# arkiven4/glow-tts

Hardware: AMD Instinct MI355X
Metric: mel_frames_per_sec_train_step (higher is better)
Workload: dtype bf16; 1 GPU; configs/base.json, LJSpeech-shaped synthetic batches, B=32/GPU, T_x<=150, T_y<=800, bf16 GEMMs; batch_per_gpu=32, T_x=150, T_y=800, batches_rotated=8, padded_frames_per_gpu_step=25600, rows_layout=ragged, graphs_captured=6, parallelism=dp1 (utterance-sharded, RCCL gradient all-reduce, fp32 on the wire), launch=one HIP graph per step (one per ragged-row bucket, captured up front)

## Files before the change

glow-tts_amd/csrc/wn_stack.hip:

```cpp
#include "common.h"
#include "internal.h"
#include "mfma_frag.h"
#include "../../include/glowtts_hip.h"

namespace {

constexpr int H = 192, TAPS = 5, NLMAX = 4;
constexpr int BM = 64;
constexpr int AP = H + 8;
constexpr int XR = BM + TAPS - 1;
constexpr int RING = 3, RING1 = RING;
constexpr int RB = 2 * RING - 1, RB1 = RB;
#ifndef WNS_PHASES
#define WNS_PHASES 0
#endif
#if WNS_PHASES
__device__ unsigned long long g_wns_ph[2 * 1024 * 48];
#define PH(i) do { if ((threadIdx.x == 0 || threadIdx.x == 256) && blockIdx.x < 1024)                                                \
                     g_wns_ph[((threadIdx.x >> 8) * 1024 + blockIdx.x) * 48 + (i)] = __builtin_amdgcn_s_memtime(); } while (0)
#else
#define PH(i) do { } while (0)
#endif
constexpr int KK2 = H / 16;
constexpr int STACK_LDS = (2 * XR + BM) * AP * 2;
constexpr int FWD_BIAS_FLOATS = NLMAX * 2 * H + (NLMAX - 1) * H;
constexpr int FWD_AFF_FLOATS = 2 * NLMAX * H;
constexpr int STACK_FWD_LDS = STACK_LDS + 2 * BM * AP * 2 + FWD_BIAS_FLOATS * 4;
constexpr int STACK_FWD_LDS_AFF = STACK_FWD_LDS + FWD_AFF_FLOATS * 4;
constexpr int CPR = H / 8;

template <typename T>
__device__ __forceinline__ const T* pinned(const T* p) { asm volatile("" : "+s"(p)); return p; }
__device__ __forceinline__ int wave_scalar()
{
  int w = __builtin_amdgcn_readfirstlane((int)(threadIdx.x >> 6));
  asm volatile("" : "+s"(w));
  return w;
}

template <typename T>
__device__ __forceinline__ T pick(T const (&arr)[NLMAX], int i)
{
  return i == 0 ? arr[0] : (i == 1 ? arr[1] : (i == 2 ? arr[2] : arr[3]));
}

template <int COND, bool DROP, int NBM, bool SAVE = true>
__global__ __launch_bounds__(256) void gt_wn_stack_fwd_kernel(gt_wn_stack_fwd_args a, uint32_t drop_thresh, float drop_scale)
{
  constexpr int BMv = 32 * NBM, XRv = BMv + TAPS - 1;
  constexpr int RINGv = NBM == 1 ? RING1 : RING;
  extern __shared__ __attribute__((aligned(16))) unsigned char smem[];
  const unsigned long long t_begin = stamp_begin(a);
  PH(0);
  const uint32_t seed_x = a.seed_dev ? *a.seed_dev : 0u;
  const int lane = threadIdx.x & 63, wave = threadIdx.x >> 6;
  const int r = lane & 31, h = lane >> 5;
  const int n_layers = a.n_layers, R = a.R;
  const int halo = 2 * (n_layers - 1);
  const int own = BMv - 2 * halo;
  const int s0 = blockIdx.x * own - halo;
  bf16_t* Xc = reinterpret_cast<bf16_t*>(smem);
  bf16_t* Xn = Xc + XR * AP;
  bf16_t* At = Xn + XR * AP;
  bf16_t* Tl = At + BM * AP;
  bf16_t* Sl = Tl + BM * AP;
  float* Bs = reinterpret_cast<float*>(Sl + BM * AP);
  constexpr int KS = H / 16, NBT = 2 * H / 32, NIT = 3 * TAPS;

  uint4 ring[RINGv][4][3];
  float rm2;
  auto w_frag = [&](const bf16_t* W, int it, int ks, int bn) {
    const int kg = it / TAPS, tap = it - kg * TAPS;
    return ldfrag_global(W, (tap * NBT + 3 * wave + bn) * KS + kg * 4 + ks, lane);
  };
  auto w_load_l = [&](const bf16_t* W, int it, uint4 (&dst)[4][3]) {
#pragma unroll
    for (int ks = 0; ks < 4; ++ks)
#pragma unroll
      for (int bn = 0; bn < 3; ++bn) dst[ks][bn] = w_frag(W, it, ks, bn);
  };
  {
    const bf16_t* x0 = static_cast<const bf16_t*>(a.x0);
    constexpr int NX = (XR * CPR + 255) / 256, NB = (FWD_BIAS_FLOATS / 4 + 255) / 256;
    uint4 xin[NX];
    float4 bin[NB];
    float4 ain[(FWD_AFF_FLOATS / 4 + 255) / 256];
    if (COND == 2) {
      const int O = H * n_layers;
#pragma unroll
      for (int i = 0; i < (FWD_AFF_FLOATS / 4 + 255) / 256; ++i) {
        const int idx = threadIdx.x + 256 * i;
        ain[i] = make_float4(0.f, 0.f, 0.f, 0.f);
        if (idx < O / 4) ain[i] = reinterpret_cast<const float4*>(a.aff_w)[idx];
        else if (idx < 2 * O / 4) ain[i] = reinterpret_cast<const float4*>(a.aff_b)[idx - O / 4];
      }
    }
#pragma unroll
    for (int i = 0; i < NX; ++i) {
      const int chunk = threadIdx.x + 256 * i, u = chunk / CPR, c8 = chunk - u * CPR, gm = s0 - 2 + u;
      xin[i] = make_uint4(0, 0, 0, 0);
      if (u < XRv && gm >= 0 && gm < R) xin[i] = *reinterpret_cast<const uint4*>(x0 + (size_t)gm * H + c8 * 8);
    }
#pragma unroll
    for (int i = 0; i < NB; ++i) {
      const int idx = threadIdx.x + 256 * i;
      bin[i] = make_float4(0.f, 0.f, 0.f, 0.f);
      if (idx < NLMAX * 2 * H / 4) {
        const int l = idx / (2 * H / 4), o = idx - l * (2 * H / 4);
        if (l < n_layers) bin[i] = reinterpret_cast<const float4*>(pick(a.b_in, l))[o];
      } else if (idx < FWD_BIAS_FLOATS / 4) {
        const int q = idx - NLMAX * 2 * H / 4, l = q / (H / 4), o = q - l * (H / 4);
        if (l < n_layers - 1) bin[i] = reinterpret_cast<const float4*>(pick(a.b_res, l))[o];
      }
    }
    {
      const int m = s0 + 32 * (wave >> 1) + r;
      rm2 = (m >= 0 && m < R) ? a.rowmask[m] : 0.0f;
    }
    {
      const bf16_t* W10 = static_cast<const bf16_t*>(a.w_in[0]);
#pragma unroll
      for (int p = 0; p < RINGv - 1; ++p) w_load_l(W10, p, ring[p]);
    }
#pragma unroll
    for (int i = 0; i < NX; ++i) {
      const int chunk = threadIdx.x + 256 * i, u = chunk / CPR, c8 = chunk - u * CPR;
      if (u < XRv) *reinterpret_cast<uint4*>(Xc + u * AP + c8 * 8) = xin[i];
    }
#pragma unroll
    for (int i = 0; i < NB; ++i) {
      const int idx = threadIdx.x + 256 * i;
      if (idx < FWD_BIAS_FLOATS / 4) reinterpret_cast<float4*>(Bs)[idx] = bin[i];
    }
    if (COND == 2) {
#pragma unroll
      for (int i = 0; i < (FWD_AFF_FLOATS / 4 + 255) / 256; ++i) {
        const int idx = threadIdx.x + 256 * i;
        if (idx < 2 * H * n_layers / 4) reinterpret_cast<float4*>(Bs + FWD_BIAS_FLOATS)[idx] = ain[i];
      }
    }
    if (threadIdx.x < 4 * 24) {
      const int q = threadIdx.x / 24, c8 = threadIdx.x - q * 24, u = q < 2 ? q : XRv - 4 + q;
      *reinterpret_cast<uint4*>(Xn + u * AP + c8 * 8) = make_uint4(0, 0, 0, 0);
    }
  }
  __syncthreads();
  PH(1);

  int cb[NBM] = {};
  float sg[NBM][2] = {};
  if (COND == 1) {
#pragma unroll
    for (int bm = 0; bm < NBM; ++bm) {
      const int m = s0 + 32 * bm + r, mc = m < 0 ? 0 : (m >= R ? R - 1 : m);
      cb[bm] = a.B > 0 ? gt_row_batch(a.row0, a.B, mc, a.Tp) : mc;
    }
  }
  if (COND == 2) {
#pragma unroll
    for (int bm = 0; bm < NBM; ++bm) {
      const int m = s0 + 32 * bm + r;
      if (m >= 0 && m < R) { const float2 v = *reinterpret_cast<const float2*>(a.aff_sig + 2 * (size_t)m); sg[bm][0] = v.x; sg[bm][1] = v.y; }
    }
  }

  for (int layer = 0; layer < n_layers; ++layer) {
    const bool last = layer == n_layers - 1;
    const bf16_t* W1 = static_cast<const bf16_t*>(pick(a.w_in, layer));
    const bf16_t* W2 = static_cast<const bf16_t*>(pick(a.w_res, layer));
    const float* bias1 = Bs + layer * 2 * H;
    const float* bias2 = Bs + NLMAX * 2 * H + layer * H;
    bf16_t* Tt = static_cast<bf16_t*>(pick(a.gate_t, layer));
    bf16_t* Ss = static_cast<bf16_t*>(pick(a.gate_s, layer));
    bf16_t* xo = static_cast<bf16_t*>(pick(a.x_out, layer));
    const uint32_t seed = (a.drop_seed + (uint32_t)layer) ^ seed_x;

    f32x16_t acc[3][NBM];
    acc_zero(acc);

    auto w_load = [&](int it, uint4 (&dst)[4][3]) { w_load_l(W1, it, dst); };
#pragma unroll
    for (int it = 0; it < NIT; ++it) {
      const int kg = it / TAPS, tap = it - kg * TAPS;
      w_load(it + RINGv - 1 < NIT ? it + RINGv - 1 : NIT - 1, ring[(it + RINGv - 1) % RINGv]);
      __builtin_amdgcn_sched_barrier(0);
      const bf16_t* xsb = Xc + (r + tap) * AP + 8 * h + kg * 64;
#pragma unroll
      for (int ks = 0; ks < 4; ++ks) {
        bf16x8_t bx[NBM];
#pragma unroll
        for (int bm = 0; bm < NBM; ++bm) bx[bm] = *reinterpret_cast<const bf16x8_t*>(xsb + 32 * bm * AP + ks * 16);
#pragma unroll
        for (int bn = 0; bn < 3; ++bn)
#pragma unroll
          for (int bm = 0; bm < NBM; ++bm)
            acc[bn][bm] = __builtin_amdgcn_mfma_f32_32x32x16_bf16(asfrag(ring[it % RINGv][ks][bn]), bx[bm], acc[bn][bm], 0, 0, 0);
      }
      __builtin_amdgcn_sched_barrier(0);
    }

    PH(2 + 6 * layer);
    int tid_e = threadIdx.x;
    asm volatile("" : "+v"(tid_e));
    const int r_e = tid_e & 31, h_e = (tid_e >> 5) & 1, wave_e = tid_e >> 6;
    const int wn2 = wave & 1, wm2 = wave >> 1;
    const bool st2 = wm2 < NBM;
    constexpr int R2 = KK2 / 2;
    uint4 ring2[R2][3];
    if (!last && st2) {
#pragma unroll
      for (int kk = 0; kk < R2; ++kk)
#pragma unroll
        for (int bn = 0; bn < 3; ++bn) ring2[kk][bn] = ldfrag_global(W2, (3 * wn2 + bn) * KK2 + kk, lane);
    }

    bf16_t* acts = static_cast<bf16_t*>(a.acts) + layer * H;
    const float* cond = COND == 1 ? a.cond + (size_t)layer * 2 * H : nullptr;
    const int aff_O = H * n_layers, aff_par = (2 * H * layer) / aff_O, aff_off = (2 * H * layer) - aff_par * aff_O;
    const float* Aw = Bs + FWD_BIAS_FLOATS + aff_off;
    const float* Ab = Aw + aff_O;
#pragma unroll
    for (int bn = 0; bn < 3; ++bn)
#pragma unroll
      for (int g = 0; g < 2; ++g) {
        const int c = 16 * (3 * wave_e + bn) + 8 * g + 4 * h_e;
        const float4 bt = *reinterpret_cast<const float4*>(bias1 + c), bs = *reinterpret_cast<const float4*>(bias1 + H + c);
        const float btv[4] = {bt.x, bt.y, bt.z, bt.w}, bsv[4] = {bs.x, bs.y, bs.z, bs.w};
#pragma unroll
        for (int bm = 0; bm < NBM; ++bm) {
          const int t = 32 * bm + r_e, m = s0 + t;
          float ctv[4] = {}, csv[4] = {};
          if (COND == 1) {
            const float* cp = cond + (size_t)cb[bm] * a.ldc + c;
            const float4 ct = *reinterpret_cast<const float4*>(cp), cs = *reinterpret_cast<const float4*>(cp + H);
            ctv[0] = ct.x; ctv[1] = ct.y; ctv[2] = ct.z; ctv[3] = ct.w; csv[0] = cs.x; csv[1] = cs.y; csv[2] = cs.z; csv[3] = cs.w;
          }
          if (COND == 2) {
            const float pv = aff_par ? sg[bm][1] : sg[bm][0];
            const float4 wt = *reinterpret_cast<const float4*>(Aw + c), ws = *reinterpret_cast<const float4*>(Aw + H + c);
            const float4 bt2 = *reinterpret_cast<const float4*>(Ab + c), bs2 = *reinterpret_cast<const float4*>(Ab + H + c);
            ctv[0] = bt2.x + pv * wt.x; ctv[1] = bt2.y + pv * wt.y; ctv[2] = bt2.z + pv * wt.z; ctv[3] = bt2.w + pv * wt.w;
            csv[0] = bs2.x + pv * ws.x; csv[1] = bs2.y + pv * ws.y; csv[2] = bs2.z + pv * ws.z; csv[3] = bs2.w + pv * ws.w;
          }
          float tt[4], ss[4], aa[4];
#pragma unroll
          for (int j = 0; j < 4; ++j) {
            float vt = acc[bn][bm][4 * g + j] + btv[j], vs = acc[bn][bm][4 * g + j + 8] + bsv[j];
            if (DROP) {
              bool kt, ks;
              drop_keep_gate(seed, m, c + j, drop_thresh16(drop_thresh), kt, ks);
              vt = kt ? vt * drop_scale : 0.0f;
              vs = ks ? vs * drop_scale : 0.0f;
            }
            vt += ctv[j]; vs += csv[j];
            tt[j] = tanhf_(vt); ss[j] = sigmoidf_(vs); aa[j] = tt[j] * ss[j];
          }
          if (SAVE) {
            *reinterpret_cast<uint2*>(Tl + t * AP + c) = pack4(tt[0], tt[1], tt[2], tt[3]);
            *reinterpret_cast<uint2*>(Sl + t * AP + c) = pack4(ss[0], ss[1], ss[2], ss[3]);
          }
          *reinterpret_cast<uint2*>(At + t * AP + c) = pack4(aa[0], aa[1], aa[2], aa[3]);
        }
      }
    PH(3 + 6 * layer);
    __syncthreads();
    PH(4 + 6 * layer);
    auto store_gate_tiles = [&]() {
      constexpr int NC = (BM * CPR + 255) / 256, NP = 2;
#pragma unroll 1
      for (int i0 = 0; i0 < NC; i0 += NP) {
        uint4 vt[NP], vs[NP], va[NP];
#pragma unroll
        for (int i = 0; i < NP; ++i) {
          const int idx = tid_e + 256 * (i0 + i), row = idx / CPR, c8 = idx - row * CPR, t = halo + row;
          vt[i] = vs[i] = va[i] = make_uint4(0, 0, 0, 0);
          if (idx < own * CPR) {
            if (SAVE) { vt[i] = *reinterpret_cast<const uint4*>(Tl + t * AP + c8 * 8); vs[i] = *reinterpret_cast<const uint4*>(Sl + t * AP + c8 * 8); }
            va[i] = *reinterpret_cast<const uint4*>(At + t * AP + c8 * 8);
          }
        }
#pragma unroll
        for (int i = 0; i < NP; ++i) {
          const int idx = tid_e + 256 * (i0 + i), row = idx / CPR, c8 = idx - row * CPR, m = s0 + halo + row;
          if (idx < own * CPR && m < R) {
            if (SAVE) {
              *reinterpret_cast<uint4*>(Tt + (size_t)m * H + c8 * 8) = vt[i];
              *reinterpret_cast<uint4*>(Ss + (size_t)m * H + c8 * 8) = vs[i];
            }
            *reinterpret_cast<uint4*>(acts + (size_t)m * a.ldacts + c8 * 8) = va[i];
          }
        }
      }
    };
    if (last) store_gate_tiles();
    if (last) break;

    f32x16_t acc2[3];
    acc_zero(acc2);
    if (st2) {
      const bf16_t* ab = At + (32 * wm2 + r) * AP + 8 * h;
#pragma unroll
      for (int kk = 0; kk < KK2; ++kk) {
        const bf16x8_t bfm = *reinterpret_cast<const bf16x8_t*>(ab + kk * 16);
#pragma unroll
        for (int bn = 0; bn < 3; ++bn) {
          acc2[bn] = __builtin_amdgcn_mfma_f32_32x32x16_bf16(asfrag(ring2[kk % R2][bn]), bfm, acc2[bn], 0, 0, 0);
          if (R2 < KK2 && kk + R2 < KK2) ring2[kk % R2][bn] = ldfrag_global(W2, (3 * wn2 + bn) * KK2 + kk + R2, lane);
        }
      }
    }
    PH(5 + 6 * layer);
    {
      const bf16_t* W1n = static_cast<const bf16_t*>(pick(a.w_in, layer + 1));
#pragma unroll
      for (int p = 0; p < RINGv - 1; ++p) w_load_l(W1n, p, ring[p]);
    }
    store_gate_tiles();
    if (st2) {
      const int t = 32 * wm2 + r;
      const float rm = rm2;
#pragma unroll
      for (int bn = 0; bn < 3; ++bn)
#pragma unroll
        for (int g = 0; g < 4; ++g) {
          const int n = 32 * (3 * wn2 + bn) + 8 * g + 4 * h;
          const float4 b2 = *reinterpret_cast<const float4*>(bias2 + n);
          float xv[4];
          unpack4(*reinterpret_cast<const uint2*>(Xc + (t + 2) * AP + n), xv);
          const uint2 v = pack4((acc2[bn][4 * g] + b2.x + xv[0]) * rm, (acc2[bn][4 * g + 1] + b2.y + xv[1]) * rm,
                                (acc2[bn][4 * g + 2] + b2.z + xv[2]) * rm, (acc2[bn][4 * g + 3] + b2.w + xv[3]) * rm);
          *reinterpret_cast<uint2*>(Xn + (t + 2) * AP + n) = v;
        }
    }
    __syncthreads();
    PH(6 + 6 * layer);
    bf16_t* tmp = Xc; Xc = Xn; Xn = tmp;
    if (SAVE) {
      constexpr int NC = (BM * CPR + 255) / 256, NP = 3;
#pragma unroll 1
      for (int i0 = 0; i0 < NC; i0 += NP) {
        uint4 vx[NP];
#pragma unroll
        for (int i = 0; i < NP; ++i) {
          const int idx = tid_e + 256 * (i0 + i), row = idx / CPR, c8 = idx - row * CPR;
          vx[i] = make_uint4(0, 0, 0, 0);
          if (idx < own * CPR) vx[i] = *reinterpret_cast<const uint4*>(Xc + (halo + row + 2) * AP + c8 * 8);
        }
#pragma unroll
        for (int i = 0; i < NP; ++i) {
          const int idx = tid_e + 256 * (i0 + i), row = idx / CPR, c8 = idx - row * CPR, m = s0 + halo + row;
          if (idx < own * CPR && m < R) *reinterpret_cast<uint4*>(xo + (size_t)m * H + c8 * 8) = vx[i];
        }
      }
    }
    if (threadIdx.x < 4 * 24) {
      const int q = threadIdx.x / 24, c8 = threadIdx.x - q * 24, u = q < 2 ? q : XRv - 4 + q;
      *reinterpret_cast<uint4*>(Xn + u * AP + c8 * 8) = make_uint4(0, 0, 0, 0);
    }
    PH(7 + 6 * layer);
  }
  PH(40);
  stamp_end(a, t_begin);
}

constexpr int BWD_THREADS = 512;
constexpr int DP = 2 * H + 8;
constexpr int EX_BYTES = 4 * 3 * 16 * 64 * 4;
constexpr int BWD_DT = XR * DP * 2;
static_assert(EX_BYTES <= BWD_DT, "the exchange buffer lives in the d pre tile");
constexpr int SBWD_LDS = BWD_DT + 4 * BM * AP * 2;

template <bool DROP>
__device__ __forceinline__ void gate_bwd4(const float (&dd)[4], const float (&t)[4], const float (&s)[4], uint32_t seed, int m, int n,
                                          uint32_t thresh, float scale, uint2& pt, uint2& ps, uint2& ct, uint2& cs)
{
  float gt[4], gs[4];
#pragma unroll
  for (int j = 0; j < 4; ++j) { gt[j] = dd[j] * s[j] * (1.0f - t[j] * t[j]); gs[j] = dd[j] * t[j] * s[j] * (1.0f - s[j]); }
  ct = pack4(gt[0], gt[1], gt[2], gt[3]); cs = pack4(gs[0], gs[1], gs[2], gs[3]);
  if (DROP) {
#pragma unroll
    for (int j = 0; j < 4; ++j) {
      bool kt, ks;
      drop_keep_gate(seed, m, n + j, drop_thresh16(thresh), kt, ks);
      gt[j] = kt ? gt[j] * scale : 0.0f;
      gs[j] = ks ? gs[j] * scale : 0.0f;
    }
  }
  pt = pack4(gt[0], gt[1], gt[2], gt[3]); ps = pack4(gs[0], gs[1], gs[2], gs[3]);
}

constexpr int B_NS = 2 * H / 64, B_NIT = B_NS * TAPS, B_KS = 2 * H / 16, B_NBT = H / 32;

template <int NB> constexpr int bwd_b0() { return NB == 2 ? 0 : 2; }

template <int NB>
__device__ __forceinline__ void bwd_w_load(const bf16_t* W1, int it, int wn, int wk, int lane, uint4 (&dst)[2][NB])
{
  const int slice = it / TAPS, tap = it - slice * TAPS;
  const bf16_t* Wt = pinned(W1 + (size_t)((tap * B_NBT + 3 * wn + bwd_b0<NB>()) * B_KS + slice * 4 + 2 * wk) * 512);
#pragma unroll
  for (int k2 = 0; k2 < 2; ++k2)
#pragma unroll
    for (int bn = 0; bn < NB; ++bn) dst[k2][bn] = ldfrag_global(Wt, bn * B_KS + k2, lane);
}
template <int RBv, int NB>
__device__ __forceinline__ void bwd_ring_prologue(const void* w, int lane, uint4 (&ring)[RBv][2][NB])
{
  const int simd = wave_scalar() & 3, wn = simd & 1, wk = simd >> 1;
  const bf16_t* W1 = pinned(static_cast<const bf16_t*>(w));
#pragma unroll
  for (int p = 0; p < RBv - 1; ++p) bwd_w_load<NB>(W1, p, wn, wk, lane, ring[p]);
}

template <int J, bool COND, bool DROP, int NBM, int NB>
__device__ __forceinline__ void bwd_step(const gt_wn_stack_bwd_args& a, uint32_t drop_thresh, float drop_scale, uint32_t seed_x,
                                         bf16_t* Dt, float* Ex, bf16_t* At, int s0, int halo,
                                         uint4 (&ring)[NBM == 1 ? RB1 : RB][2][NB], float rm)
{
  int tid = threadIdx.x;
  asm volatile("" : "+v"(tid));
  const int lane = tid & 63, r = lane & 31, h = lane >> 5;
  const int simd = wave_scalar() & 3;
  const int wn = simd & 1, wk = simd >> 1;
  constexpr int B0 = bwd_b0<NB>();
  constexpr int BMv = 32 * NBM;
  constexpr int RBv = NBM == 1 ? RB1 : RB;
  const bool act = wk < NBM;
  const int n_layers = a.n_layers, R = a.R;
  const bf16_t* via = static_cast<const bf16_t*>(a.via_skip);
  constexpr int NIT = B_NIT;
  const bf16_t* W1 = pinned(static_cast<const bf16_t*>(a.w_in_d[J]));
  f32x16_t acc[NB][NBM];
#pragma unroll
  for (int bn = 0; bn < NB; ++bn)
#pragma unroll
    for (int bm = 0; bm < NBM; ++bm)
#pragma unroll
      for (int e = 0; e < 16; ++e) acc[bn][bm][e] = 0.0f;
  auto w_load = [&](int it, uint4 (&dst)[2][NB]) { bwd_w_load<NB>(W1, it, wn, wk, lane, dst); };
#pragma unroll
  for (int it = 0; it < NIT; ++it) {
    const int slice = it / TAPS, tap = it - slice * TAPS;
    w_load(it + RBv - 1 < NIT ? it + RBv - 1 : NIT - 1, ring[(it + RBv - 1) % RBv]);
    __builtin_amdgcn_sched_barrier(0);
    const bf16_t* xsb = Dt + (r + tap) * DP + 8 * h + slice * 64 + 32 * wk;
#pragma unroll
    for (int k2 = 0; k2 < 2; ++k2) {
      bf16x8_t bx[NBM];
#pragma unroll
      for (int bm = 0; bm < NBM; ++bm) bx[bm] = *reinterpret_cast<const bf16x8_t*>(xsb + 32 * bm * DP + k2 * 16);
#pragma unroll
      for (int bn = 0; bn < NB; ++bn)
#pragma unroll
        for (int bm = 0; bm < NBM; ++bm)
          acc[bn][bm] = __builtin_amdgcn_mfma_f32_32x32x16_bf16(asfrag(ring[it % RBv][k2][bn]), bx[bm], acc[bn][bm], 0, 0, 0);
    }
    __builtin_amdgcn_sched_barrier(0);
  }
  PH(2 + 8 * (3 - J));
  constexpr int JL = J > 0 ? J - 1 : 0;
  const bf16_t* W2 = pinned(static_cast<const bf16_t*>(a.w_res_d[JL]));
  uint4 ring2[KK2][NB];
  auto w2_load = [&](int k0, int k1) {
    if (J > 0 && act) {
#pragma unroll
      for (int kk = k0; kk < k1; ++kk)
#pragma unroll
        for (int bn = 0; bn < NB; ++bn) ring2[kk][bn] = ldfrag_global(W2, (3 * wn + B0 + bn) * KK2 + kk, lane);
    }
  };
  w2_load(0, KK2 / 2);
  constexpr int JLp = J > 0 ? J - 1 : 0;
  constexpr int NPRE = (BM * CPR + BWD_THREADS - 1) / BWD_THREADS;
  uint4 pre[3][NPRE];
  if (J > 0) {
    const bf16_t* Tg = static_cast<const bf16_t*>(a.gate_t[JLp]);
    const bf16_t* Sg = static_cast<const bf16_t*>(a.gate_s[JLp]);
#pragma unroll
    for (int i = 0; i < NPRE; ++i) {
      const int idx = tid + BWD_THREADS * i, row = idx / CPR, c8 = idx - row * CPR, mm = s0 + row;
      pre[0][i] = pre[1][i] = pre[2][i] = make_uint4(0, 0, 0, 0);
      if (row < BMv && mm >= 0 && mm < R) {
        pre[0][i] = *reinterpret_cast<const uint4*>(via + (size_t)mm * a.ldvs + JLp * H + c8 * 8);
        pre[1][i] = *reinterpret_cast<const uint4*>(Tg + (size_t)mm * H + c8 * 8);
        pre[2][i] = *reinterpret_cast<const uint4*>(Sg + (size_t)mm * H + c8 * 8);
      }
    }
  }
  __syncthreads();

  if (NBM == 2 || wk) {
    float* mine = Ex + (simd * 3 + B0) * (16 * 64);
#pragma unroll
    for (int bn = 0; bn < NB; ++bn)
#pragma unroll
      for (int e = 0; e < 16; ++e) mine[(bn * 16 + e) * 64 + lane] = (NBM == 2 && !wk) ? acc[bn][NBM - 1][e] : acc[bn][0][e];
  }
  __syncthreads();
  f32x16_t sum[NB];
  if (act) {
    const float* theirs = Ex + ((simd ^ 2) * 3 + B0) * (16 * 64);
#pragma unroll
    for (int bn = 0; bn < NB; ++bn)
#pragma unroll
      for (int e = 0; e < 16; ++e) sum[bn][e] = ((NBM == 2 && wk) ? acc[bn][NBM - 1][e] : acc[bn][0][e]) + theirs[(bn * 16 + e) * 64 + lane];
  }
  w2_load(KK2 / 2, KK2);
  PH(3 + 8 * (3 - J));
  const int t = 32 * wk + r, m = s0 + t;
  const bool mine_row = act && t >= halo && t < BMv - halo && m < R;
  if (act) {
#pragma unroll
    for (int bn = 0; bn < NB; ++bn)
#pragma unroll
// ... 119 lines not shown
  const int halo = 2 * (n_layers - 1), own = BMv - 2 * halo;
  const int s0 = blockIdx.x * own - halo;
  bf16_t* Dt = reinterpret_cast<bf16_t*>(smem);
  float* Ex = reinterpret_cast<float*>(smem);
  bf16_t* At = reinterpret_cast<bf16_t*>(smem + BWD_DT);
  const bf16_t* via = static_cast<const bf16_t*>(a.via_skip);
  constexpr int RBv = NBM == 1 ? RB1 : RB;
  uint4 ring[RBv][2][NB];
  bwd_ring_prologue<RBv, NB>(pick(a.w_in_d, n_layers - 1), lane, ring);
  float rm;
  {
    const int m = s0 + 32 * (simd >> 1) + (lane & 31);
    rm = (m >= 0 && m < R) ? a.rowmask[m] : 0.0f;
  }

  {
    const int L = n_layers - 1;
    const bf16_t* Tt = static_cast<const bf16_t*>(pick(a.gate_t, L));
    const bf16_t* Ss = static_cast<const bf16_t*>(pick(a.gate_s, L));
    bf16_t* dpre = static_cast<bf16_t*>(pick(a.dpre, L));
    bf16_t* dpre_c = static_cast<bf16_t*>(pick(a.dpre_c, L));
    const uint32_t seed = (a.drop_seed + (uint32_t)L) ^ seed_x;
    constexpr int NH = (XR * CPR + BWD_THREADS - 1) / BWD_THREADS;
    uint4 hv[3][NH];
#pragma unroll
    for (int i = 0; i < NH; ++i) {
      const int idx = threadIdx.x + BWD_THREADS * i, u = idx / CPR, c8 = idx - u * CPR, m = s0 - 2 + u;
      hv[0][i] = hv[1][i] = hv[2][i] = make_uint4(0, 0, 0, 0);
      if (u < XRv && m >= 0 && m < R) {
        hv[0][i] = *reinterpret_cast<const uint4*>(via + (size_t)m * a.ldvs + L * H + c8 * 8);
        hv[1][i] = *reinterpret_cast<const uint4*>(Tt + (size_t)m * H + c8 * 8);
        hv[2][i] = *reinterpret_cast<const uint4*>(Ss + (size_t)m * H + c8 * 8);
      }
    }
#pragma unroll
    for (int i = 0; i < NH; ++i) {
      const int idx = threadIdx.x + BWD_THREADS * i, u = idx / CPR, c8 = idx - u * CPR, m = s0 - 2 + u, n = c8 * 8;
      if (u >= XRv) continue;
      uint2 pt[2], ps[2], ct[2], cs[2];
      pt[0] = pt[1] = ps[0] = ps[1] = ct[0] = ct[1] = cs[0] = cs[1] = make_uint2(0, 0);
      if (m >= 0 && m < R) {
#pragma unroll
        for (int q = 0; q < 2; ++q) {
          float dd[4], t[4], sg[4];
          unpack4(q ? make_uint2(hv[0][i].z, hv[0][i].w) : make_uint2(hv[0][i].x, hv[0][i].y), dd);
          unpack4(q ? make_uint2(hv[1][i].z, hv[1][i].w) : make_uint2(hv[1][i].x, hv[1][i].y), t);
          unpack4(q ? make_uint2(hv[2][i].z, hv[2][i].w) : make_uint2(hv[2][i].x, hv[2][i].y), sg);
          gate_bwd4<DROP>(dd, t, sg, seed, m, n + 4 * q, drop_thresh, drop_scale, pt[q], ps[q], ct[q], cs[q]);
        }
        if (u - 2 >= halo && u - 2 < BMv - halo) {
          *reinterpret_cast<uint4*>(dpre + (size_t)m * 2 * H + n) = make_uint4(pt[0].x, pt[0].y, pt[1].x, pt[1].y);
          *reinterpret_cast<uint4*>(dpre + (size_t)m * 2 * H + H + n) = make_uint4(ps[0].x, ps[0].y, ps[1].x, ps[1].y);
          if (COND) {
            *reinterpret_cast<uint4*>(dpre_c + (size_t)m * 2 * H + n) = make_uint4(ct[0].x, ct[0].y, ct[1].x, ct[1].y);
            *reinterpret_cast<uint4*>(dpre_c + (size_t)m * 2 * H + H + n) = make_uint4(cs[0].x, cs[0].y, cs[1].x, cs[1].y);
          }
        }
      }
      *reinterpret_cast<uint4*>(Dt + u * DP + n) = make_uint4(pt[0].x, pt[0].y, pt[1].x, pt[1].y);
      *reinterpret_cast<uint4*>(Dt + u * DP + H + n) = make_uint4(ps[0].x, ps[0].y, ps[1].x, ps[1].y);
    }
  }
  __syncthreads();
  PH(1);
  if (n_layers > 3) bwd_step<3, COND, DROP, NBM, NB>(a, drop_thresh, drop_scale, seed_x, Dt, Ex, At, s0, halo, ring, rm);
  if (n_layers > 2) bwd_step<2, COND, DROP, NBM, NB>(a, drop_thresh, drop_scale, seed_x, Dt, Ex, At, s0, halo, ring, rm);
  if (n_layers > 1) bwd_step<1, COND, DROP, NBM, NB>(a, drop_thresh, drop_scale, seed_x, Dt, Ex, At, s0, halo, ring, rm);
  bwd_step<0, COND, DROP, NBM, NB>(a, drop_thresh, drop_scale, seed_x, Dt, Ex, At, s0, halo, ring, rm);
  PH(40);
}

template <bool COND, bool DROP, int NBM>
__global__ __launch_bounds__(BWD_THREADS) void gt_wn_stack_bwd_kernel(gt_wn_stack_bwd_args a, uint32_t drop_thresh, float drop_scale)
{
  if (wave_scalar() < 4) bwd_wave<COND, DROP, NBM, 2>(a, drop_thresh, drop_scale);
  else bwd_wave<COND, DROP, NBM, 1>(a, drop_thresh, drop_scale);
}

}

#if WNS_PHASES
extern "C" int gt_dev_wns_phases(void* dst, size_t bytes)
{
  return hipMemcpyFromSymbol(dst, HIP_SYMBOL(g_wns_ph), bytes < sizeof(g_wns_ph) ? bytes : sizeof(g_wns_ph)) == hipSuccess ? 0 : -1;
}
#endif

#ifndef WNS_SMALL_TILE_MAX_WGS
#define WNS_SMALL_TILE_MAX_WGS 80
#endif
#ifndef WNS_SMALL_TILE_MAX_WGS_FWD
#define WNS_SMALL_TILE_MAX_WGS_FWD 98
#endif
static int stack_row_blocks(int R, int n_layers, bool fwd = false)
{
  const int own2 = BM - 4 * (n_layers - 1), own1 = 32 - 4 * (n_layers - 1);
  return (own1 >= 8 && (R + own2 - 1) / own2 <= (fwd ? WNS_SMALL_TILE_MAX_WGS_FWD : WNS_SMALL_TILE_MAX_WGS)) ? 1 : 2;
}
extern "C" int gt_wn_stack_rows_per_workgroup(int n_layers) { return BM - 4 * (n_layers - 1); }
extern "C" int gt_wn_stack_row_blocks(int R, int n_layers, int fwd) { return stack_row_blocks(R, n_layers, fwd != 0); }

extern "C" int gt_wn_stack_fwd(const gt_wn_stack_fwd_args* args, void* stream)
{
  if (!args) return GT_E_INVAL;
  const gt_wn_stack_fwd_args& a = *args;
  if (a.R < 0) return GT_E_INVAL;
  if (a.R == 0) return GT_OK;
  if (a.H != H || a.taps != TAPS || a.n_layers < 1 || a.n_layers > NLMAX) return GT_E_UNSUPPORTED;
  if (!a.x0 || !a.rowmask || !a.acts || a.ldacts < a.n_layers * H || (a.ldacts & 7) || (a.cond && (a.ldc & 3))) return GT_E_INVAL;
  if (!al16(a.x0) || !al16(a.acts) || !al16(a.cond)) return GT_E_ALIGN;
  int n_save = 0, n_given = 0;
  for (int i = 0; i < a.n_layers; ++i) {
    n_save += 2 + (i < a.n_layers - 1);
    n_given += (a.gate_t[i] != nullptr) + (a.gate_s[i] != nullptr) + (i < a.n_layers - 1 && a.x_out[i] != nullptr);
  }
  if (n_given != 0 && n_given != n_save) return GT_E_INVAL;
  const bool save = n_given != 0;
  for (int i = 0; i < a.n_layers; ++i) {
    if (!a.w_in[i] || !a.b_in[i]) return GT_E_INVAL;
    if (i < a.n_layers - 1 && (!a.w_res[i] || !a.b_res[i])) return GT_E_INVAL;
    if (!al16(a.w_in[i]) || !al16(a.b_in[i]) || !al16(a.gate_t[i]) || !al16(a.gate_s[i]) || !al16(a.w_res[i]) || !al16(a.b_res[i]) ||
        !al16(a.x_out[i])) return GT_E_ALIGN;
  }
  if (a.cond && (a.Tp <= 0 || (a.row0 && a.B <= 0))) return GT_E_INVAL;
  const bool affine = a.aff_w || a.aff_b || a.aff_sig;
  if (affine) {
    if (a.cond || !a.aff_w || !a.aff_b || !a.aff_sig || ((H * a.n_layers) % (2 * H))) return GT_E_INVAL;
    if (!al16(a.aff_w) || !al16(a.aff_b) || ((uintptr_t)a.aff_sig & 7)) return GT_E_ALIGN;
  }
  if (a.drop_p >= 1.0f) return GT_E_UNSUPPORTED;
  uint32_t thresh; float scale;
  gt_drop_params(a.drop_p, &thresh, &scale);
  typedef void (*kern_t)(gt_wn_stack_fwd_args, uint32_t, float);
  static const kern_t kerns[12] = {gt_wn_stack_fwd_kernel<0, false, 2>, gt_wn_stack_fwd_kernel<0, true, 2>, gt_wn_stack_fwd_kernel<1, false, 2>,
                                   gt_wn_stack_fwd_kernel<1, true, 2>, gt_wn_stack_fwd_kernel<2, false, 2>, gt_wn_stack_fwd_kernel<2, true, 2>,
                                   gt_wn_stack_fwd_kernel<0, false, 1>, gt_wn_stack_fwd_kernel<0, true, 1>, gt_wn_stack_fwd_kernel<1, false, 1>,
                                   gt_wn_stack_fwd_kernel<1, true, 1>, gt_wn_stack_fwd_kernel<2, false, 1>, gt_wn_stack_fwd_kernel<2, true, 1>};
  static const kern_t kerns_nosave[4] = {gt_wn_stack_fwd_kernel<0, false, 2, false>, gt_wn_stack_fwd_kernel<1, false, 2, false>,
                                         gt_wn_stack_fwd_kernel<0, false, 1, false>, gt_wn_stack_fwd_kernel<1, false, 1, false>};
  if (!save && (thresh || affine)) return GT_E_UNSUPPORTED;
  static bool attr = false;
  if (!attr) {
    for (int i = 0; i < 12; ++i)
      if (hipFuncSetAttribute(reinterpret_cast<const void*>(kerns[i]), hipFuncAttributeMaxDynamicSharedMemorySize,
                              (i % 6) >= 4 ? STACK_FWD_LDS_AFF : STACK_FWD_LDS) != hipSuccess)
        return GT_E_LAUNCH;
    for (int i = 0; i < 4; ++i)
      if (hipFuncSetAttribute(reinterpret_cast<const void*>(kerns_nosave[i]), hipFuncAttributeMaxDynamicSharedMemorySize, STACK_FWD_LDS) != hipSuccess)
        return GT_E_LAUNCH;
    attr = true;
  }
  const int nbm = stack_row_blocks(a.R, a.n_layers, true);
  const int own = 32 * nbm - 4 * (a.n_layers - 1);
  const dim3 grid((a.R + own - 1) / own), block(256);
  const int mode = affine ? 2 : (a.cond ? 1 : 0);
  const kern_t kern = save ? kerns[(nbm == 1 ? 6 : 0) + 2 * mode + (thresh ? 1 : 0)] : kerns_nosave[(nbm == 1 ? 2 : 0) + mode];
  hipLaunchKernelGGL(kern, grid, block, affine ? STACK_FWD_LDS_AFF : STACK_FWD_LDS, static_cast<hipStream_t>(stream), a, thresh, scale);
  return gt_launch_status(__func__);
}

extern "C" int gt_wn_stack_bwd(const gt_wn_stack_bwd_args* args, void* stream)
{
  if (!args) return GT_E_INVAL;
  const gt_wn_stack_bwd_args& a = *args;
  if (a.R < 0) return GT_E_INVAL;
  if (a.R == 0) return GT_OK;
  if (a.H != H || a.taps != TAPS || a.n_layers < 1 || a.n_layers > NLMAX) return GT_E_UNSUPPORTED;
  if (!a.via_skip || !a.rowmask || a.ldvs < a.n_layers * H || (a.ldvs & 7)) return GT_E_INVAL;
  if (!al16(a.via_skip)) return GT_E_ALIGN;
  for (int i = 0; i < a.n_layers; ++i) {
    if (!a.w_in_d[i] || !a.gate_t[i] || !a.gate_s[i] || !a.dpre[i] || !a.dx[i]) return GT_E_INVAL;
    if (i < a.n_layers - 1 && !a.w_res_d[i]) return GT_E_INVAL;
    if (!al16(a.w_in_d[i]) || !al16(a.gate_t[i]) || !al16(a.gate_s[i]) || !al16(a.dpre[i]) || !al16(a.dpre_c[i]) || !al16(a.dx[i]) ||
        !al16(a.w_res_d[i])) return GT_E_ALIGN;
  }
  if (a.drop_p >= 1.0f) return GT_E_UNSUPPORTED;
  uint32_t thresh; float scale;
  gt_drop_params(a.drop_p, &thresh, &scale);
  bool cond = false;
  for (int i = 0; i < a.n_layers; ++i) cond = cond || a.dpre_c[i];
  for (int i = 0; i < a.n_layers; ++i) if (cond && !a.dpre_c[i]) return GT_E_INVAL;
  typedef void (*kern_t)(gt_wn_stack_bwd_args, uint32_t, float);
  static const kern_t kerns[8] = {gt_wn_stack_bwd_kernel<false, false, 2>, gt_wn_stack_bwd_kernel<false, true, 2>,
                                  gt_wn_stack_bwd_kernel<true, false, 2>, gt_wn_stack_bwd_kernel<true, true, 2>,
                                  gt_wn_stack_bwd_kernel<false, false, 1>, gt_wn_stack_bwd_kernel<false, true, 1>,
                                  gt_wn_stack_bwd_kernel<true, false, 1>, gt_wn_stack_bwd_kernel<true, true, 1>};
  static bool attr = false;
  if (!attr) {
    for (kern_t k : kerns)
      if (hipFuncSetAttribute(reinterpret_cast<const void*>(k), hipFuncAttributeMaxDynamicSharedMemorySize, SBWD_LDS) != hipSuccess)
        return GT_E_LAUNCH;
    attr = true;
  }
  const int nbm = stack_row_blocks(a.R, a.n_layers);
  const int own = 32 * nbm - 4 * (a.n_layers - 1);
  const dim3 grid((a.R + own - 1) / own), block(BWD_THREADS);
  hipLaunchKernelGGL(kerns[(nbm == 1 ? 4 : 0) + (cond ? 2 : 0) + (thresh ? 1 : 0)], grid, block, SBWD_LDS, static_cast<hipStream_t>(stream), a, thresh, scale);
  return gt_launch_status(__func__);
}
```

Measured before the change: 4.866 million mel-frames/s.

## Split WN stack forward across 512 threads with 2+1 column-block wave halves

The fused WaveNet-stack forward kernel goes from 256 to 512 threads. Each SIMD's three output column blocks are split between two waves: waves 0-3 take two blocks, waves 4-7 take one. Weight prefetch now works in half-steps with a deeper ring, the residual-weight loads are split around the gate epilogue, and the layer loop is unrolled at compile time over four constant-index layer steps. The aim is more waves per CU to hide global weight-load and MFMA latency and to shorten per-wave serial work, at the cost of uneven load between the two wave halves and more register/LDS contention.

```diff
diff --git a/glow-tts_amd/csrc/wn_stack.hip b/glow-tts_amd/csrc/wn_stack.hip
--- a/glow-tts_amd/csrc/wn_stack.hip
+++ b/glow-tts_amd/csrc/wn_stack.hip
@@ -9,7 +9,7 @@
 constexpr int BM = 64;
 constexpr int AP = H + 8;
 constexpr int XR = BM + TAPS - 1;
-constexpr int RING = 3, RING1 = RING;
+constexpr int RING = 3;
 constexpr int RB = 2 * RING - 1, RB1 = RB;
 #ifndef WNS_PHASES
 #define WNS_PHASES 0
@@ -44,17 +44,45 @@
   return i == 0 ? arr[0] : (i == 1 ? arr[1] : (i == 2 ? arr[2] : arr[3]));
 }
 
-template <int COND, bool DROP, int NBM, bool SAVE = true>
-__global__ __launch_bounds__(256) void gt_wn_stack_fwd_kernel(gt_wn_stack_fwd_args a, uint32_t drop_thresh, float drop_scale)
+constexpr int FWD_THREADS = 512;
+constexpr int F_KS = H / 16, F_NBT = 2 * H / 32, F_NHS = 2 * 3 * TAPS;
+
+template <int NB> constexpr int fwd_b0() { return NB == 2 ? 0 : 2; }
+
+template <int NB>
+__device__ __forceinline__ void fwd_w_load(const bf16_t* W1, int hs, int simd, int lane, uint4 (&dst)[2][NB])
+{
+  const int it = hs >> 1, kg = it / TAPS, tap = it - kg * TAPS;
+  const bf16_t* Wt = pinned(W1 + (size_t)((tap * F_NBT + 3 * simd + fwd_b0<NB>()) * F_KS + kg * 4 + 2 * (hs & 1)) * 512);
+#pragma unroll
+  for (int k2 = 0; k2 < 2; ++k2)
+#pragma unroll
+    for (int bn = 0; bn < NB; ++bn) dst[k2][bn] = ldfrag_global(Wt, bn * F_KS + k2, lane);
+}
+template <int RBv, int NB>
+__device__ __forceinline__ void fwd_ring_prologue(const void* w, int lane, uint4 (&ring)[RBv][2][NB])
+{
+  const int simd = wave_scalar() & 3;
+  const bf16_t* W1 = pinned(static_cast<const bf16_t*>(w));
+#pragma unroll
+  for (int p = 0; p < RBv - 1; ++p) fwd_w_load<NB>(W1, p, simd, lane, ring[p]);
+}
+
+template <int J> struct layer_ic { static constexpr int value = J; };
+static_assert(NLMAX == 4, "fwd_wave spells out four layer steps");
+
+template <int COND, bool DROP, int NBM, bool SAVE, int NB>
+__device__ __forceinline__ void fwd_wave(const gt_wn_stack_fwd_args& a, uint32_t drop_thresh, float drop_scale)
 {
   constexpr int BMv = 32 * NBM, XRv = BMv + TAPS - 1;
-  constexpr int RINGv = NBM == 1 ? RING1 : RING;
+  constexpr int RBv = NBM == 1 ? RB1 : RB;
+  constexpr int B0 = fwd_b0<NB>();
   extern __shared__ __attribute__((aligned(16))) unsigned char smem[];
   const unsigned long long t_begin = stamp_begin(a);
   PH(0);
   const uint32_t seed_x = a.seed_dev ? *a.seed_dev : 0u;
-  const int lane = threadIdx.x & 63, wave = threadIdx.x >> 6;
-  const int r = lane & 31, h = lane >> 5;
+  const int lane = threadIdx.x & 63, simd = (threadIdx.x >> 6) & 3;
+  const int r = lane & 31;
   const int n_layers = a.n_layers, R = a.R;
   const int halo = 2 * (n_layers - 1);
   const int own = BMv - 2 * halo;
@@ -65,31 +93,22 @@
   bf16_t* Tl = At + BM * AP;
   bf16_t* Sl = Tl + BM * AP;
   float* Bs = reinterpret_cast<float*>(Sl + BM * AP);
-  constexpr int KS = H / 16, NBT = 2 * H / 32, NIT = 3 * TAPS;
-
-  uint4 ring[RINGv][4][3];
+  constexpr int NHS = F_NHS;
+
+  uint4 ring[RBv][2][NB];
   float rm2;
-  auto w_frag = [&](const bf16_t* W, int it, int ks, int bn) {
-    const int kg = it / TAPS, tap = it - kg * TAPS;
-    return ldfrag_global(W, (tap * NBT + 3 * wave + bn) * KS + kg * 4 + ks, lane);
-  };
-  auto w_load_l = [&](const bf16_t* W, int it, uint4 (&dst)[4][3]) {
-#pragma unroll
-    for (int ks = 0; ks < 4; ++ks)
-#pragma unroll
-      for (int bn = 0; bn < 3; ++bn) dst[ks][bn] = w_frag(W, it, ks, bn);
-  };
   {
     const bf16_t* x0 = static_cast<const bf16_t*>(a.x0);
-    constexpr int NX = (XR * CPR + 255) / 256, NB = (FWD_BIAS_FLOATS / 4 + 255) / 256;
+    constexpr int NX = (XR * CPR + FWD_THREADS - 1) / FWD_THREADS, NBI = (FWD_BIAS_FLOATS / 4 + FWD_THREADS - 1) / FWD_THREADS;
+    constexpr int NAF = (FWD_AFF_FLOATS / 4 + FWD_THREADS - 1) / FWD_THREADS;
     uint4 xin[NX];
-    float4 bin[NB];
-    float4 ain[(FWD_AFF_FLOATS / 4 + 255) / 256];
+    float4 bin[NBI];
+    float4 ain[NAF];
     if (COND == 2) {
       const int O = H * n_layers;
 #pragma unroll
-      for (int i = 0; i < (FWD_AFF_FLOATS / 4 + 255) / 256; ++i) {
-        const int idx = threadIdx.x + 256 * i;
+      for (int i = 0; i < NAF; ++i) {
+        const int idx = threadIdx.x + FWD_THREADS * i;
         ain[i] = make_float4(0.f, 0.f, 0.f, 0.f);
         if (idx < O / 4) ain[i] = reinterpret_cast<const float4*>(a.aff_w)[idx];
         else if (idx < 2 * O / 4) ain[i] = reinterpret_cast<const float4*>(a.aff_b)[idx - O / 4];
@@ -97,13 +116,13 @@
     }
 #pragma unroll
     for (int i = 0; i < NX; ++i) {
-      const int chunk = threadIdx.x + 256 * i, u = chunk / CPR, c8 = chunk - u * CPR, gm = s0 - 2 + u;
+      const int chunk = threadIdx.x + FWD_THREADS * i, u = chunk / CPR, c8 = chunk - u * CPR, gm = s0 - 2 + u;
       xin[i] = make_uint4(0, 0, 0, 0);
       if (u < XRv && gm >= 0 && gm < R) xin[i] = *reinterpret_cast<const uint4*>(x0 + (size_t)gm * H + c8 * 8);
     }
 #pragma unroll
-    for (int i = 0; i < NB; ++i) {
-      const int idx = threadIdx.x + 256 * i;
+    for (int i = 0; i < NBI; ++i) {
+      const int idx = threadIdx.x + FWD_THREADS * i;
       bin[i] = make_float4(0.f, 0.f, 0.f, 0.f);
       if (idx < NLMAX * 2 * H / 4) {
         const int l = idx / (2 * H / 4), o = idx - l * (2 * H / 4);
@@ -114,33 +133,29 @@
       }
     }
     {
-      const int m = s0 + 32 * (wave >> 1) + r;
+      const int m = s0 + 32 * (simd >> 1) + r;
       rm2 = (m >= 0 && m < R) ? a.rowmask[m] : 0.0f;
     }
-    {
-      const bf16_t* W10 = static_cast<const bf16_t*>(a.w_in[0]);
-#pragma unroll
-      for (int p = 0; p < RINGv - 1; ++p) w_load_l(W10, p, ring[p]);
-    }
+    fwd_ring_prologue<RBv, NB>(a.w_in[0], lane, ring);
 #pragma unroll
     for (int i = 0; i < NX; ++i) {
-      const int chunk = threadIdx.x + 256 * i, u = chunk / CPR, c8 = chunk - u * CPR;
+      const int chunk = threadIdx.x + FWD_THREADS * i, u = chunk / CPR, c8 = chunk - u * CPR;
       if (u < XRv) *reinterpret_cast<uint4*>(Xc + u * AP + c8 * 8) = xin[i];
     }
 #pragma unroll
-    for (int i = 0; i < NB; ++i) {
-      const int idx = threadIdx.x + 256 * i;
+    for (int i = 0; i < NBI; ++i) {
+      const int idx = threadIdx.x + FWD_THREADS * i;
       if (idx < FWD_BIAS_FLOATS / 4) reinterpret_cast<float4*>(Bs)[idx] = bin[i];
     }
     if (COND == 2) {
 #pragma unroll
-      for (int i = 0; i < (FWD_AFF_FLOATS / 4 + 255) / 256; ++i) {
-        const int idx = threadIdx.x + 256 * i;
+      for (int i = 0; i < NAF; ++i) {
+        const int idx = threadIdx.x + FWD_THREADS * i;
         if (idx < 2 * H * n_layers / 4) reinterpret_cast<float4*>(Bs + FWD_BIAS_FLOATS)[idx] = ain[i];
       }
     }
-    if (threadIdx.x < 4 * 24) {
-      const int q = threadIdx.x / 24, c8 = threadIdx.x - q * 24, u = q < 2 ? q : XRv - 4 + q;
+    if (NB == 1 && threadIdx.x < 256 + 4 * 24) {
+      const int z = threadIdx.x - 256, q = z / 24, c8 = z - q * 24, u = q < 2 ? q : XRv - 4 + q;
       *reinterpret_cast<uint4*>(Xn + u * AP + c8 * 8) = make_uint4(0, 0, 0, 0);
     }
   }
@@ -164,10 +179,9 @@
     }
   }
 
-  for (int layer = 0; layer < n_layers; ++layer) {
-    const bool last = layer == n_layers - 1;
-    const bf16_t* W1 = static_cast<const bf16_t*>(pick(a.w_in, layer));
-    const bf16_t* W2 = static_cast<const bf16_t*>(pick(a.w_res, layer));
+  auto layer_step = [&](auto layer_c) __attribute__((always_inline)) -> bool {
+    constexpr int layer = decltype(layer_c)::value;
+    const bool last = layer == NLMAX - 1 || layer == n_layers - 1;
     const float* bias1 = Bs + layer * 2 * H;
     const float* bias2 = Bs + NLMAX * 2 * H + layer * H;
     bf16_t* Tt = static_cast<bf16_t*>(pick(a.gate_t, layer));
@@ -175,44 +189,61 @@
     bf16_t* xo = static_cast<bf16_t*>(pick(a.x_out, layer));
     const uint32_t seed = (a.drop_seed + (uint32_t)layer) ^ seed_x;
 
-    f32x16_t acc[3][NBM];
-    acc_zero(acc);
-
-    auto w_load = [&](int it, uint4 (&dst)[4][3]) { w_load_l(W1, it, dst); };
-#pragma unroll
-    for (int it = 0; it < NIT; ++it) {
-      const int kg = it / TAPS, tap = it - kg * TAPS;
-      w_load(it + RINGv - 1 < NIT ? it + RINGv - 1 : NIT - 1, ring[(it + RINGv - 1) % RINGv]);
-      __builtin_amdgcn_sched_barrier(0);
-      const bf16_t* xsb = Xc + (r + tap) * AP + 8 * h + kg * 64;
-#pragma unroll
-      for (int ks = 0; ks < 4; ++ks) {
-        bf16x8_t bx[NBM];
-#pragma unroll
-        for (int bm = 0; bm < NBM; ++bm) bx[bm] = *reinterpret_cast<const bf16x8_t*>(xsb + 32 * bm * AP + ks * 16);
-#pragma unroll
-        for (int bn = 0; bn < 3; ++bn)
-#pragma unroll
-          for (int bm = 0; bm < NBM; ++bm)
-            acc[bn][bm] = __builtin_amdgcn_mfma_f32_32x32x16_bf16(asfrag(ring[it % RINGv][ks][bn]), bx[bm], acc[bn][bm], 0, 0, 0);
-      }
-      __builtin_amdgcn_sched_barrier(0);
+    f32x16_t acc[NB][NBM];
+#pragma unroll
+    for (int bn = 0; bn < NB; ++bn)
+#pragma unroll
+      for (int bm = 0; bm < NBM; ++bm)
+#pragma unroll
+        for (int e = 0; e < 16; ++e) acc[bn][bm][e] = 0.0f;
+    {
+      int tid_k = threadIdx.x;
+      asm volatile("" : "+v"(tid_k));
+      const int lane_k = tid_k & 63, r_k = lane_k & 31, h_k = lane_k >> 5;
+      const int simd_k = wave_scalar() & 3;
+      const bf16_t* W1 = pinned(static_cast<const bf16_t*>(pick(a.w_in, layer)));
+#pragma unroll
+      for (int hs = 0; hs < NHS; ++hs) {
+        const int it = hs >> 1, kg = it / TAPS, tap = it - kg * TAPS;
+        if (hs + RBv - 1 < NHS) fwd_w_load<NB>(W1, hs + RBv - 1, simd_k, lane_k, ring[(hs + RBv - 1) % RBv]);
+        __builtin_amdgcn_sched_barrier(0);
+        const bf16_t* xsb = Xc + (r_k + tap) * AP + 8 * h_k + kg * 64 + 32 * (hs & 1);
+#pragma unroll
+        for (int k2 = 0; k2 < 2; ++k2) {
+          bf16x8_t bx[NBM];
+#pragma unroll
+          for (int bm = 0; bm < NBM; ++bm) bx[bm] = *reinterpret_cast<const bf16x8_t*>(xsb + 32 * bm * AP + k2 * 16);
+#pragma unroll
+          for (int bn = 0; bn < NB; ++bn)
+#pragma unroll
+            for (int bm = 0; bm < NBM; ++bm)
+              acc[bn][bm] = __builtin_amdgcn_mfma_f32_32x32x16_bf16(asfrag(ring[hs % RBv][k2][bn]), bx[bm], acc[bn][bm], 0, 0, 0);
+        }
+#pragma unroll
+        for (int bn = 0; bn < NB; ++bn)
+#pragma unroll
+          for (int bm = 0; bm < NBM; ++bm) asm volatile("" : "+v"(acc[bn][bm]));
+        __builtin_amdgcn_sched_barrier(0);
+      }
     }
 
     PH(2 + 6 * layer);
     int tid_e = threadIdx.x;
     asm volatile("" : "+v"(tid_e));
-    const int r_e = tid_e & 31, h_e = (tid_e >> 5) & 1, wave_e = tid_e >> 6;
-    const int wn2 = wave & 1, wm2 = wave >> 1;
+    const int lane_e = tid_e & 63, r_e = tid_e & 31, h_e = (tid_e >> 5) & 1, simd_e = (tid_e >> 6) & 3;
+    const int simd2 = wave_scalar() & 3, wn2 = simd2 & 1, wm2 = simd2 >> 1;
     const bool st2 = wm2 < NBM;
-    constexpr int R2 = KK2 / 2;
-    uint4 ring2[R2][3];
-    if (!last && st2) {
-#pragma unroll
-      for (int kk = 0; kk < R2; ++kk)
-#pragma unroll
-        for (int bn = 0; bn < 3; ++bn) ring2[kk][bn] = ldfrag_global(W2, (3 * wn2 + bn) * KK2 + kk, lane);
-    }
+    uint4 ring2[KK2][NB];
+    auto w2_load = [&](int k0, int k1) {
+      if (!last && st2) {
+        const bf16_t* W2 = pinned(static_cast<const bf16_t*>(pick(a.w_res, layer)));
+#pragma unroll
+        for (int kk = k0; kk < k1; ++kk)
+#pragma unroll
+          for (int bn = 0; bn < NB; ++bn) ring2[kk][bn] = ldfrag_global(W2, (3 * wn2 + B0 + bn) * KK2 + kk, lane_e);
+      }
+    };
+    w2_load(0, KK2 / 2);
 
     bf16_t* acts = static_cast<bf16_t*>(a.acts) + layer * H;
     const float* cond = COND == 1 ? a.cond + (size_t)layer * 2 * H : nullptr;
@@ -220,10 +251,10 @@
     const float* Aw = Bs + FWD_BIAS_FLOATS + aff_off;
     const float* Ab = Aw + aff_O;
 #pragma unroll
-    for (int bn = 0; bn < 3; ++bn)
+    for (int bn = 0; bn < NB; ++bn)
 #pragma unroll
       for (int g = 0; g < 2; ++g) {
-        const int c = 16 * (3 * wave_e + bn) + 8 * g + 4 * h_e;
+        const int c = 16 * (3 * simd_e + B0 + bn) + 8 * g + 4 * h_e;
         const float4 bt = *reinterpret_cast<const float4*>(bias1 + c), bs = *reinterpret_cast<const float4*>(bias1 + H + c);
         const float btv[4] = {bt.x, bt.y, bt.z, bt.w}, bsv[4] = {bs.x, bs.y, bs.z, bs.w};
 #pragma unroll
@@ -260,19 +291,20 @@
             *reinterpret_cast<uint2*>(Sl + t * AP + c) = pack4(ss[0], ss[1], ss[2], ss[3]);
           }
           *reinterpret_cast<uint2*>(At + t * AP + c) = pack4(aa[0], aa[1], aa[2], aa[3]);
-        }
-      }
+          __builtin_amdgcn_sched_barrier(0);
+        }
+      }
+    w2_load(KK2 / 2, KK2);
     PH(3 + 6 * layer);
     __syncthreads();
     PH(4 + 6 * layer);
     auto store_gate_tiles = [&]() {
-      constexpr int NC = (BM * CPR + 255) / 256, NP = 2;
-#pragma unroll 1
-      for (int i0 = 0; i0 < NC; i0 += NP) {
+      constexpr int NP = (BM * CPR + FWD_THREADS - 1) / FWD_THREADS;
+      {
         uint4 vt[NP], vs[NP], va[NP];
 #pragma unroll
         for (int i = 0; i < NP; ++i) {
-          const int idx = tid_e + 256 * (i0 + i), row = idx / CPR, c8 = idx - row * CPR, t = halo + row;
+          const int idx = tid_e + FWD_THREADS * i, row = idx / CPR, c8 = idx - row * CPR, t = halo + row;
           vt[i] = vs[i] = va[i] = make_uint4(0, 0, 0, 0);
           if (idx < own * CPR) {
             if (SAVE) { vt[i] = *reinterpret_cast<const uint4*>(Tl + t * AP + c8 * 8); vs[i] = *reinterpret_cast<const uint4*>(Sl + t * AP + c8 * 8); }
@@ -281,7 +313,7 @@
         }
 #pragma unroll
         for (int i = 0; i < NP; ++i) {
-          const int idx = tid_e + 256 * (i0 + i), row = idx / CPR, c8 = idx - row * CPR, m = s0 + halo + row;
+          const int idx = tid_e + FWD_THREADS * i, row = idx / CPR, c8 = idx - row * CPR, m = s0 + halo + row;
           if (idx < own * CPR && m < R) {
             if (SAVE) {
               *reinterpret_cast<uint4*>(Tt + (size_t)m * H + c8 * 8) = vt[i];
@@ -292,38 +324,31 @@
         }
       }
     };
-    if (last) store_gate_tiles();
-    if (last) break;
-
-    f32x16_t acc2[3];
+    if (last) { store_gate_tiles(); return true; }
+
+    f32x16_t acc2[NB];
     acc_zero(acc2);
     if (st2) {
-      const bf16_t* ab = At + (32 * wm2 + r) * AP + 8 * h;
+      const bf16_t* ab = At + (32 * wm2 + r_e) * AP + 8 * h_e;
 #pragma unroll
       for (int kk = 0; kk < KK2; ++kk) {
         const bf16x8_t bfm = *reinterpret_cast<const bf16x8_t*>(ab + kk * 16);
 #pragma unroll
-        for (int bn = 0; bn < 3; ++bn) {
-          acc2[bn] = __builtin_amdgcn_mfma_f32_32x32x16_bf16(asfrag(ring2[kk % R2][bn]), bfm, acc2[bn], 0, 0, 0);
-          if (R2 < KK2 && kk + R2 < KK2) ring2[kk % R2][bn] = ldfrag_global(W2, (3 * wn2 + bn) * KK2 + kk + R2, lane);
-        }
+        for (int bn = 0; bn < NB; ++bn)
+          acc2[bn] = __builtin_amdgcn_mfma_f32_32x32x16_bf16(asfrag(ring2[kk][bn]), bfm, acc2[bn], 0, 0, 0);
       }
     }
     PH(5 + 6 * layer);
-    {
-      const bf16_t* W1n = static_cast<const bf16_t*>(pick(a.w_in, layer + 1));
-#pragma unroll
-      for (int p = 0; p < RINGv - 1; ++p) w_load_l(W1n, p, ring[p]);
-    }
+    fwd_ring_prologue<RBv, NB>(pick(a.w_in, layer + 1), lane_e, ring);
     store_gate_tiles();
     if (st2) {
-      const int t = 32 * wm2 + r;
+      const int t = 32 * wm2 + r_e;
       const float rm = rm2;
 #pragma unroll
-      for (int bn = 0; bn < 3; ++bn)
+      for (int bn = 0; bn < NB; ++bn)
 #pragma unroll
         for (int g = 0; g < 4; ++g) {
-          const int n = 32 * (3 * wn2 + bn) + 8 * g + 4 * h;
+          const int n = 32 * (3 * wn2 + B0 + bn) + 8 * g + 4 * h_e;
           const float4 b2 = *reinterpret_cast<const float4*>(bias2 + n);
           float xv[4];
           unpack4(*reinterpret_cast<const uint2*>(Xc + (t + 2) * AP + n), xv);
@@ -336,31 +361,43 @@
     PH(6 + 6 * layer);
     bf16_t* tmp = Xc; Xc = Xn; Xn = tmp;
     if (SAVE) {
-      constexpr int NC = (BM * CPR + 255) / 256, NP = 3;
-#pragma unroll 1
-      for (int i0 = 0; i0 < NC; i0 += NP) {
+      constexpr int NP = (BM * CPR + FWD_THREADS - 1) / FWD_THREADS;
+      {
         uint4 vx[NP];
 #pragma unroll
         for (int i = 0; i < NP; ++i) {
-          const int idx = tid_e + 256 * (i0 + i), row = idx / CPR, c8 = idx - row * CPR;
+          const int idx = tid_e + FWD_THREADS * i, row = idx / CPR, c8 = idx - row * CPR;
           vx[i] = make_uint4(0, 0, 0, 0);
           if (idx < own * CPR) vx[i] = *reinterpret_cast<const uint4*>(Xc + (halo + row + 2) * AP + c8 * 8);
         }
 #pragma unroll
         for (int i = 0; i < NP; ++i) {
-          const int idx = tid_e + 256 * (i0 + i), row = idx / CPR, c8 = idx - row * CPR, m = s0 + halo + row;
+          const int idx = tid_e + FWD_THREADS * i, row = idx / CPR, c8 = idx - row * CPR, m = s0 + halo + row;
           if (idx < own * CPR && m < R) *reinterpret_cast<uint4*>(xo + (size_t)m * H + c8 * 8) = vx[i];
         }
       }
     }
-    if (threadIdx.x < 4 * 24) {
-      const int q = threadIdx.x / 24, c8 = threadIdx.x - q * 24, u = q < 2 ? q : XRv - 4 + q;
+    if (NB == 1 && tid_e < 256 + 4 * 24) {
+      const int z = tid_e - 256, q = z / 24, c8 = z - q * 24, u = q < 2 ? q : XRv - 4 + q;
       *reinterpret_cast<uint4*>(Xn + u * AP + c8 * 8) = make_uint4(0, 0, 0, 0);
     }
     PH(7 + 6 * layer);
-  }
+    return false;
+  };
+  if (!layer_step(layer_ic<0>{}) && !layer_step(layer_ic<1>{}) && !layer_step(layer_ic<2>{})) layer_step(layer_ic<3>{});
   PH(40);
-  stamp_end(a, t_begin);
+  if (a.stamps && (threadIdx.x & 255) == 0) {
+    unsigned long long* slot = a.stamps + 2 * (a.stamp_slot + (a.stamp_base ? *a.stamp_base : 0));
+    if (blockIdx.x == 0 && threadIdx.x == 0) slot[0] = t_begin;
+    atomicMax(slot + 1, (unsigned long long)wall_clock64());
+  }
+}
+
+template <int COND, bool DROP, int NBM, bool SAVE = true>
+__global__ __launch_bounds__(FWD_THREADS) void gt_wn_stack_fwd_kernel(gt_wn_stack_fwd_args a, uint32_t drop_thresh, float drop_scale)
+{
+  if (wave_scalar() < 4) fwd_wave<COND, DROP, NBM, SAVE, 2>(a, drop_thresh, drop_scale);
+  else fwd_wave<COND, DROP, NBM, SAVE, 1>(a, drop_thresh, drop_scale);
 }
 
 constexpr int BWD_THREADS = 512;
@@ -786,7 +823,7 @@
   }
   const int nbm = stack_row_blocks(a.R, a.n_layers, true);
   const int own = 32 * nbm - 4 * (a.n_layers - 1);
-  const dim3 grid((a.R + own - 1) / own), block(256);
+  const dim3 grid((a.R + own - 1) / own), block(FWD_THREADS);
   const int mode = affine ? 2 : (a.cond ? 1 : 0);
   const kern_t kern = save ? kerns[(nbm == 1 ? 6 : 0) + 2 * mode + (thresh ? 1 : 0)] : kerns_nosave[(nbm == 1 ? 2 : 0) + mode];
   hipLaunchKernelGGL(kern, grid, block, affine ? STACK_FWD_LDS_AFF : STACK_FWD_LDS, static_cast<hipStream_t>(stream), a, thresh, scale);
```

After: 4.900 million mel-frames/s, median of 6. About the same (+0.7%).
